# 0x002A/MuCHSALSA

Hardware: AMD Instinct MI355X
Metric: overlap-pairs/s (higher is better)
Workload: dtype int32+f64; 1 GPU; 100k synthetic Nanopore x10 kb, 500k unitig anchors, 10x coverage (BASELINE.json configs[2]); rows=5059558, reads=100000, anchors=499992, edges=981460, edgematches_rank0=25532466, orders_rank0=1029308, parallelism=one job on one GPU, edges_proven_clean_rank0=5372

## Files before the change

include/msgpu.h:

```cpp
#ifndef MSGPU_H
#define MSGPU_H

#include <stddef.h>
#include <stdint.h>

#ifdef __cplusplus
extern "C" {
#endif

#define MSGPU_VERSION 1

#define MSGPU_OK 0
#define MSGPU_E_IO (-1)
#define MSGPU_E_FORMAT (-2)
#define MSGPU_E_NUMBER (-3)
#define MSGPU_E_NOMEM (-4)
#define MSGPU_E_ARG (-5)
#define MSGPU_E_HIP (-6)
#define MSGPU_E_STATE (-7)
#define MSGPU_E_IDS (-8)
#define MSGPU_E_NODEVICE (-9)
#define MSGPU_E_LAYOUT (-10)
#define MSGPU_E_TIMEOUT (-11)

// ... 149 lines not shown
int msgpu_load_rows(msgpu_ctx *ctx, const msgpu_row *rows, size_t n_rows);
int msgpu_load_rows_packed(msgpu_ctx *ctx, const msgpu_packed_rows *packed);
int msgpu_load_rows_device(msgpu_ctx *ctx, const void *d_rows, size_t n_rows);


int msgpu_calculate_edges(msgpu_ctx *ctx);


int msgpu_chaining_and_overlaps(msgpu_ctx *ctx);


int msgpu_get_counts(msgpu_ctx *ctx, msgpu_counts *out);
int msgpu_get_timings(msgpu_ctx *ctx, msgpu_timings *out);
int msgpu_get_chain_band_counts(msgpu_ctx *ctx, uint64_t *n_banded, uint64_t *n_fallback);
int msgpu_chain_band_width(void);
int msgpu_set_stage_events(msgpu_ctx *ctx, int on);

int msgpu_copy_tables(msgpu_ctx *ctx, msgpu_edge *edges, msgpu_edgematch *ems, msgpu_order *orders, uint32_t *ids);
int msgpu_copy_tables_device(msgpu_ctx *ctx, void *d_edges, void *d_ems, void *d_orders, void *d_ids);
int msgpu_copy_reads(msgpu_ctx *ctx, int32_t *read_len, uint32_t *read_first_line);

int msgpu_merge_gathered(msgpu_ctx *ctx, const void *d_gathered, uint32_t world, const uint64_t *counts,
                         uint64_t slab_bytes, uint64_t off_edges, uint64_t off_orders, uint64_t off_ids, void *d_edges,
                         void *d_orders, void *d_ids);

int msgpu_merge_gathered_ex(msgpu_ctx *ctx, const void *d_gathered, uint32_t world, const uint64_t *counts,
                            uint64_t slab_bytes, uint64_t off_edges, uint64_t off_orders, uint64_t off_ids,
                            const uint32_t *id_base, void *d_edges, void *d_orders, void *d_ids, void *hip_stream);

uint64_t msgpu_wire_edges_bytes(uint64_t n_edges);
// ... 709 lines not shown
```

muchsalsa_amd/_lib.py:

```python
import ctypes as C
import os

import numpy as np

_HERE = os.path.dirname(os.path.abspath(__file__))
LIB_PATH = os.environ.get("MSGPU_LIB") or os.path.join(_HERE, "libmsgpu.so")

ROW_DTYPE = np.dtype([("anchor_id", "<u4"), ("read_id", "<u4"), ("read_len", "<i4"), ("i_lo", "<i4"),
                      ("i_hi", "<i4"), ("n_lo", "<i4"), ("n_hi", "<i4"), ("score", "<u4"), ("line", "<u4"),
                      ("flags", "<u4")])
EDGE_DTYPE = np.dtype([("v1", "<u4"), ("v2", "<u4"), ("em_off", "<u8"), ("order_off", "<u8"), ("em_cnt", "<u4"),
                       ("order_cnt", "<u2"), ("shadow", "u1"), ("pad", "u1")])
EM_DTYPE = np.dtype([("ov_lo", "<i4"), ("ov_hi", "<i4"), ("score", "<f8"), ("anchor_id", "<u4"), ("line", "<u4"),
                     ("flags", "<u4"), ("edge_idx", "<u4")])
ORDER_DTYPE = np.dtype([("edge_idx", "<u4"), ("flags", "<u4"), ("left_offset", "<f8"), ("right_offset", "<f8"),
                        ("score", "<u8"), ("ids_off", "<u8"), ("ids_cnt", "<u4"), ("start", "<u4"), ("end", "<u4"),
                        ("base", "<u4"), ("pad", "<u4", (2,))])
COPY_DTYPE = np.dtype([("src_off", "<u8"), ("dst_off", "<u8"), ("len", "<u4"), ("flags", "<u4")])
assert (ROW_DTYPE.itemsize, EDGE_DTYPE.itemsize, EM_DTYPE.itemsize, ORDER_DTYPE.itemsize) == (40, 32, 32, 64)
assert COPY_DTYPE.itemsize == 24
COPY_ILLUMINA, COPY_REVCOMP = 1, 2
PATH_READ_DTYPE = np.dtype([("read_id", "<u4"), ("direction", "<u4"), ("nanopore_length", "<u8")])
PATH_ORDER_DTYPE = np.dtype([("score", "<u8"), ("base_read", "<u4"), ("ids_off", "<u4"), ("ids_cnt", "<u4"),
                             ("pad", "<u4")])
# ... 297 lines not shown
    ("msgpu_paf_rows", C.c_void_p, [C.c_void_p, C.POINTER(C.c_size_t)]),
    ("msgpu_paf_line_count", C.c_size_t, [C.c_void_p]),
    ("msgpu_paf_read_count", C.c_uint32, [C.c_void_p]),
    ("msgpu_paf_anchor_count", C.c_uint32, [C.c_void_p]),
    ("msgpu_paf_read_name", C.c_char_p, [C.c_void_p, C.c_uint32]),
    ("msgpu_paf_anchor_name", C.c_char_p, [C.c_void_p, C.c_uint32]),
    ("msgpu_paf_register_sequences", C.c_int, [C.c_void_p, C.c_int, C.c_void_p, C.c_void_p, C.POINTER(C.c_uint32)]),
    ("msgpu_load_rows", C.c_int, [C.c_void_p, C.c_void_p, C.c_size_t]),
    ("msgpu_load_rows_device", C.c_int, [C.c_void_p, C.c_void_p, C.c_size_t]),
    ("msgpu_calculate_edges", C.c_int, [C.c_void_p]),
    ("msgpu_chaining_and_overlaps", C.c_int, [C.c_void_p]),
    ("msgpu_get_counts", C.c_int, [C.c_void_p, C.POINTER(Counts)]),
    ("msgpu_get_timings", C.c_int, [C.c_void_p, C.POINTER(Timings)]),
    ("msgpu_get_chain_band_counts", C.c_int, [C.c_void_p, C.POINTER(C.c_uint64), C.POINTER(C.c_uint64)]),
    ("msgpu_chain_band_width", C.c_int, []),
    ("msgpu_set_stage_events", C.c_int, [C.c_void_p, C.c_int]),
    ("msgpu_copy_tables", C.c_int, [C.c_void_p, C.c_void_p, C.c_void_p, C.c_void_p, C.c_void_p]),
    ("msgpu_copy_tables_device", C.c_int, [C.c_void_p, C.c_void_p, C.c_void_p, C.c_void_p, C.c_void_p]),
    ("msgpu_copy_reads", C.c_int, [C.c_void_p, C.c_void_p, C.c_void_p]),
    ("msgpu_merge_gathered", C.c_int, [C.c_void_p, C.c_void_p, C.c_uint32, C.c_void_p, C.c_uint64, C.c_uint64,
                                       C.c_uint64, C.c_uint64, C.c_void_p, C.c_void_p, C.c_void_p]),
    ("msgpu_merge_gathered_ex", C.c_int, [C.c_void_p, C.c_void_p, C.c_uint32, C.c_void_p, C.c_uint64, C.c_uint64,
                                          C.c_uint64, C.c_uint64, C.c_void_p, C.c_void_p, C.c_void_p, C.c_void_p,
                                          C.c_void_p]),
    ("msgpu_wire_edges_bytes", C.c_uint64, [C.c_uint64]),
    ("msgpu_wire_orders_bytes", C.c_uint64, [C.c_uint64]),
    ("msgpu_wire_ids_bytes", C.c_uint64, [C.c_uint64, C.c_uint32]),
    ("msgpu_pack_wire", C.c_int, [C.c_void_p, C.c_void_p, C.c_void_p, C.c_void_p, C.c_uint32]),
    ("msgpu_merge_wire", C.c_int, [C.c_void_p, C.c_void_p, C.c_uint32, C.c_void_p, C.c_uint64, C.c_uint64, C.c_uint64,
                                   C.c_uint64, C.c_uint32, C.c_void_p, C.c_void_p, C.c_void_p, C.c_void_p, C.c_void_p]),
# ... 274 lines not shown
```

muchsalsa_amd/csrc/msgpu_api.hip:

```cpp
#include <hip/hip_runtime.h>

#include <chrono>
#include <cmath>
#include <cstdarg>
#include <cstdio>
#include <cstdlib>
#include <cstring>
#include <condition_variable>
#include <deque>
#include <mutex>
#include <new>
#include <thread>
#include <vector>
#include <algorithm>
#include <sys/mman.h>
#include <unistd.h>

#include "asm_internal.h"
#include "host_pool.h"
#include "msgpu.h"
#include "msgpu_internal.h"
#include "msgpu_stage.h"

using namespace msgpu;
// ... 1162 lines not shown
int msgpu_get_chain_band_counts(msgpu_ctx *c, uint64_t *n_banded, uint64_t *n_fallback) {
  if (!c || !n_banded || !n_fallback) return MSGPU_E_ARG;
  *n_banded = *n_fallback = 0;
  if (c->state < ST_CHAINED || !c->chain_chunks.p) return MSGPU_OK;
  STAGE_HIP(c, hipSetDevice(c->device));
  const size_t n_chunks = static_cast<size_t>((c->chain_E + COMPACT_CHUNK - 1) / COMPACT_CHUNK);
  const size_t fb_word  = 2 * static_cast<size_t>(c->chain_E / COMPACT_CHUNK + 1);
  std::vector<unsigned long long> w(fb_word + 1);
  STAGE_HIP(c, hipStreamSynchronize(c->stream));
  STAGE_HIP(c, hipMemcpy(w.data(), c->chain_chunks.p, w.size() * 8, hipMemcpyDeviceToHost));
  for (size_t k = 0; k < n_chunks; ++k) *n_banded += (w[2 * k] >> 16) & 0xffffull;
  *n_fallback = w[fb_word];
  return MSGPU_OK;
}

int msgpu_get_timings(msgpu_ctx *c, msgpu_timings *out) {
  if (!c || !out) return MSGPU_E_ARG;
  memset(out, 0, sizeof(*out));
  STAGE_HIP(c, hipStreamSynchronize(c->stream));
  if (c->have_index_t) STAGE_HIP(c, hipEventElapsedTime(&out->index_ms, c->ev[0], c->ev[1]));
  if (c->have_cand_t) STAGE_HIP(c, hipEventElapsedTime(&out->candidates_ms, c->ev[2], c->ev[3]));
  if (c->have_chain_t) {
    if (c->have_stage_t) {
      STAGE_HIP(c, hipEventElapsedTime(&out->chain_ms, c->ev[4], c->ev[7]));
      STAGE_HIP(c, hipEventElapsedTime(&out->compact_ms, c->ev[7], c->ev[8]));
    }
    double   sum = 0;
    uint32_t n   = 0;
    for (uint32_t i = 0; i < c->ck_count; ++i) {
      const uint32_t slot = (c->ck_head + msgpu_ctx::CK_RING - 1 - i) % msgpu_ctx::CK_RING;
// ... 717 lines not shown
```

muchsalsa_amd/csrc/msgpu_device.h:

```cpp
#ifndef MSGPU_DEVICE_H
#define MSGPU_DEVICE_H

#include <hip/hip_runtime.h>
#include <stdint.h>

#include "msgpu.h"
#include "msgpu_internal.h"

namespace msgpu {

__device__ __forceinline__ IRow load_irow(const IRow *p) {
  const uint4 *q = reinterpret_cast<const uint4 *>(p);
  uint4        a = q[0], b = q[1];
  IRow         r;
  r.n_lo  = static_cast<int>(a.x);
  r.n_hi  = static_cast<int>(a.y);
  r.i_lo  = static_cast<int>(a.z);
  r.i_hi  = static_cast<int>(a.w);
  r.score = b.x;
  r.line  = b.y;
  r.other = b.z;
  r.pf    = b.w;
  return r;
}
// ... 155 lines not shown
    x = static_cast<long long>((static_cast<unsigned long long>(hi[0]) << 32) | lo[0]);
    y = static_cast<long long>((static_cast<unsigned long long>(hi[1]) << 32) | lo[1]);
    v = x > y ? x : y;
  }
  return v;
}
__device__ __forceinline__ double wave_prefix_max_f64(double v) {
  v = dpp_max_step<0x111>(v);
  v = dpp_max_step<0x112>(v);
  v = dpp_max_step<0x114>(v);
  v = dpp_max_step<0x118>(v);
  v = dpp_max_step<0x142, 0xa>(v);
  v = dpp_max_step<0x143, 0xc>(v);
  return v;
}

template <int NT> __device__ __forceinline__ uint32_t block_excl_scan(uint32_t v, uint32_t *s_wave , uint32_t *total) {
  const int      lane = threadIdx.x & 63, wave = threadIdx.x >> 6;
  const uint32_t inc  = wave_incl_scan(v);
  if (lane == 63) s_wave[wave] = inc;
  __syncthreads();
  uint32_t base = 0, tot = 0;
#pragma unroll
  for (int w = 0; w < NT / 64; ++w) {
    const uint32_t x = s_wave[w];
    base += w < wave ? x : 0u;
    tot += x;
  }
  *total = tot;
  __syncthreads();
// ... 110 lines not shown
```

muchsalsa_amd/csrc/msgpu_internal.h:

```cpp
#ifndef MSGPU_INTERNAL_H
#define MSGPU_INTERNAL_H

#include <hip/hip_runtime.h>
#include <stdint.h>

#include "msgpu.h"

namespace msgpu {

struct IRow {
  int32_t  n_lo, n_hi, i_lo, i_hi;
  uint32_t score, line, other, pf;
};
static_assert(sizeof(IRow) == 32, "IRow must be 32 bytes");
struct SRow {
  int32_t  i_lo, i_hi;
  uint32_t read, pf;
};
static_assert(sizeof(SRow) == 16, "SRow must be 16 bytes");
constexpr uint32_t PF_POS_MASK = 0x3fffffffu;
constexpr uint32_t PF_DIR      = 1u << 30;
constexpr uint32_t PF_PRIM     = 1u << 31;

enum { SC_MAXIDS = 0 , SC_ERR = 1, SC_TOTAL_A = 2, SC_TOTAL_B = 3, SC_TOTAL_C = 4, SC_NLISTS = 5 ,
// ... 220 lines not shown
void launch_classify_reads(hipStream_t st, const uint32_t *read_off, const uint32_t *read_cnt, const uint32_t *bound,
                           const uint64_t *cand_off, uint32_t V, uint32_t shard, uint32_t nshards, uint32_t lo,
                           uint32_t hi, CandDesc *l0, CandDesc *l1, CandDesc *l2, uint32_t *l3, uint32_t *n_lists, const CandZero &z,
                           unsigned long long *own_total = nullptr);
void launch_candidates(hipStream_t st, const CandArgs &a, int cls, const CandDesc *list, uint32_t n_list);
void launch_candidates_big(hipStream_t st, const CandArgs &a, const uint32_t *list, uint32_t n_list, uint64_t *big_key,
                           uint32_t *big_t, uint32_t *big_r2s, uint32_t *big_pfx);
void launch_emit_edges(hipStream_t st, const EmitArgs &a, bool reduce);
constexpr uint32_t PAIR_TAB_STRIDE = 2016 + 128;
#ifndef MSGPU_CHAIN_BAND
#define MSGPU_CHAIN_BAND 12
#endif
static_assert(MSGPU_CHAIN_BAND >= 1 && MSGPU_CHAIN_BAND <= 62, "band width");
constexpr int chain_band_pairs(int n) { return MSGPU_CHAIN_BAND * (MSGPU_CHAIN_BAND + 1) / 2 + (n - 1 - MSGPU_CHAIN_BAND) * MSGPU_CHAIN_BAND; }
static_assert(chain_band_pairs(64) <= 2016, "the band table fits the stride of the others");
constexpr uint32_t PAIR_TAB_BAND64_OFF = 4 * PAIR_TAB_STRIDE + 2 * PAIR_TAB_STRIDE + 3 * 2 * PAIR_TAB_STRIDE;
constexpr uint32_t PAIR_TAB_WORDS      = PAIR_TAB_BAND64_OFF + 2 * PAIR_TAB_STRIDE;
constexpr int CHAIN_FAST_SHORTCUT = 1, CHAIN_FAST_BAND = 2;
void launch_fill_pair_tab(hipStream_t st, uint32_t *tab);
void launch_chain(hipStream_t st, const ChainArgs &a, const uint32_t *list, uint32_t n_list);
void launch_chain_sub(hipStream_t st, const ChainArgs &a, int width, const uint32_t *list, uint32_t n_list);
struct ChainSubLists {
  const uint32_t *list32, *list16, *list8;
  uint32_t        n32, n16, n8, nb32, nb16;
};
void launch_chain_sub_all(hipStream_t st, const ChainArgs &a, const uint32_t *l32, uint32_t n32, const uint32_t *l16, uint32_t n16,
                          const uint32_t *l8, uint32_t n8);
size_t big_elem_bytes();
size_t big_path_bytes();
void launch_chain_big(hipStream_t st, const ChainArgs &a, const uint32_t *big_list, const uint64_t *big_off,
                      uint32_t n_big, void *elems, void *paths);
void launch_merge_gathered(hipStream_t st, const MergeArgs &a);
// ... 35 lines not shown
```

muchsalsa_amd/csrc/msgpu_kernels.hip:

```cpp
#include <hip/hip_runtime.h>
#include <stdint.h>
#include <stdlib.h>

#include <type_traits>
#include <utility>

#include "msgpu.h"
#include "msgpu_internal.h"
#include "msgpu_device.h"

namespace msgpu {


constexpr int SCAN_ITEMS = 8;
uint32_t      scan_blocks(uint64_t n);

template <class T> __global__ __launch_bounds__(256) void k_scan_reduce(const uint32_t *in, uint64_t n, T *block_sums) {
  __shared__ T s[4];
  uint64_t     base = static_cast<uint64_t>(blockIdx.x) * 256 * SCAN_ITEMS;
  T            sum  = 0;
  for (int i = 0; i < SCAN_ITEMS; ++i) {
    uint64_t idx = base + static_cast<uint64_t>(i) * 256 + threadIdx.x;
    if (idx < n) sum += in[idx];
  }
// ... 1279 lines not shown
        a.big_off[i]  = atomicAdd(&a.big_cursor[1], static_cast<unsigned long long>(ed.em_cnt));
      } else if (ed.em_cnt) {
        a.list[atomicAdd(&s_pos[ed.em_cnt - 1], 1u)] = static_cast<uint32_t>(eb + e);
      }
    }
  }
}
void launch_emit_edges(hipStream_t st, const EmitArgs &a, bool reduce) {
  if (reduce && a.n_chunks)
    hipLaunchKernelGGL(k_cand_reduce, dim3(a.n_chunks), dim3(1024), 0, st, a.n_edge, a.n_cand, a.cand_off, a.edge_scr_start, a.V,
                       const_cast<unsigned long long *>(a.chunk_sums), const_cast<uint32_t *>(a.hist));
  hipLaunchKernelGGL(k_emit_edges, dim3(a.n_chunks ? a.n_chunks : 1), dim3(1024), 0, st, a);
}


__device__ __forceinline__ void chunk_add(unsigned long long *chunk_sums, uint64_t e, bool clean, uint32_t n_orders, uint32_t n_ids, bool banded = false) {
  static_assert(COMPACT_CHUNK < (1u << 16), "two 16-bit edge counts in the low half of a chunk sum");
  unsigned long long *c = chunk_sums + 2 * (e / COMPACT_CHUNK);
  __hip_atomic_fetch_add(c, (clean ? 1ull : 0ull) | (banded ? 1ull << 16 : 0ull) | (static_cast<unsigned long long>(n_orders) << 32), __ATOMIC_RELAXED, __HIP_MEMORY_SCOPE_AGENT);
  __hip_atomic_fetch_add(c + 1, static_cast<unsigned long long>(n_ids), __ATOMIC_RELAXED, __HIP_MEMORY_SCOPE_AGENT);
}
__device__ __forceinline__ void edge_counts(msgpu_edge *edges, uint64_t e, uint32_t em_cnt, uint32_t n_orders, uint32_t n_ids, bool shadow) {
  reinterpret_cast<uint4 *>(&edges[e])[1] = make_uint4(n_ids, 0u, em_cnt, (n_orders & 0xffffu) | (shadow ? 1u << 16 : 0u));
}
__device__ __forceinline__ void band_fallback_add(unsigned long long *chunk_sums, uint64_t n_edges) {
  __hip_atomic_fetch_add(chunk_sums + 2 * (n_edges / COMPACT_CHUNK + 1), 1ull, __ATOMIC_RELAXED, __HIP_MEMORY_SCOPE_AGENT);
}

struct PathRec {
  uint64_t mask;
  uint64_t score;
  uint32_t primary;
  uint32_t pad;
};

struct __attribute__((aligned(16))) ChainElem {
  double clo1, chi1;
  double clo2, chi2;
  int    rlo1, rhi1, rlo2, rhi2;
};

// ... 646 lines not shown
  const int      wave = threadIdx.x >> 6, lane = threadIdx.x & 63;
  const int      g = lane / W, sl = lane % W, gbase = g * W;
  const uint32_t slot    = (block * 4 + wave) * G + g;
  const bool     valid_g = slot < n_list;
  if (__ballot(valid_g) == 0) return;
  const uint32_t   e  = valid_g ? list[slot] : list[0];
  const msgpu_edge ed = a.edges[e];
  const uint32_t   n  = (valid_g && ed.em_cnt <= static_cast<uint32_t>(W)) ? ed.em_cnt : 0u;
  const uint64_t   cp = a.edge_cand[e];
  const bool       act = sl < static_cast<int>(n);
  const uint32_t   v1 = ed.v1, v2 = ed.v2;
  const uint32_t   n1 = a.read_cnt[v1], n2 = a.read_cnt[v2];
  const int        len1 = a.read_len[v1], len2 = a.read_len[v2];
  ChainElem       *el = reinterpret_cast<ChainElem *>(s_wavebuf[wave]);
  uint32_t        *cm = s_cm[wave];

  uint32_t  j1 = 0, q2 = 0, anchor = 0;
  double    clo1 = 0, clo2 = 0, ovr1 = 0, ovr2 = 0, em_score = 0;
  bool      em_dir = false, em_prim = false;
  ChainElem x{};
  cm[lane] = 0;
  if (act) {
    j1            = a.cand_j[cp + sl];
    const uint32_t qt = a.cand_q[cp + sl];
    const IRow m1 = load_irow(&a.by_read[a.read_off[v1] + j1]);
    const IRow m2 = load_irow(&a.by_read[a.read_off[v2] + qt]);
    anchor        = m1.other;
    const int  ov_lo = max(m1.i_lo, m2.i_lo), ov_hi = min(m1.i_hi, m2.i_hi);
    const bool d1 = (m1.pf & PF_DIR) != 0, d2 = (m2.pf & PF_DIR) != 0;
    em_dir           = d1 == d2;
// ... 76 lines not shown
      int a_hi = act ? static_cast<int>(ceil(av)) : -2147483647 - 1;
      int a_lo = act ? static_cast<int>(floor(av)) : 2147483647;
      int b_hi = act ? static_cast<int>(ceil(bv)) : -2147483647 - 1;
      int b_lo = act ? static_cast<int>(floor(bv)) : 2147483647;
#pragma unroll
      for (int d = W / 2; d > 0; d >>= 1) {
        a_hi = max(a_hi, __shfl_xor(a_hi, d));
        a_lo = min(a_lo, __shfl_xor(a_lo, d));
        b_hi = max(b_hi, __shfl_xor(b_hi, d));
        b_lo = min(b_lo, __shfl_xor(b_lo, d));
      }
      clean = maybe && static_cast<long long>(a_hi) - b_lo <= a.fast_margin && static_cast<long long>(b_hi) - a_lo <= a.fast_margin;
    }
  }

  const int P = clean ? 0 : static_cast<int>(n * (n - 1) / 2);
  const int nP   = longest_prefix<W>(__ballot(act && !clean));
  const int Pmax = nP * (nP - 1) / 2;
  const bool               one_dir = __ballot(m_plus != 0 && m_minus != 0) == 0;
  const unsigned long long KD_one  = __ballot(m_minus == 0);
  static_assert(sizeof(ChainElem) == 48, "the pair table holds byte offsets of 48-byte elements");
  const __amdgpu_buffer_rsrc_t tab_rsrc = __builtin_amdgcn_make_buffer_rsrc(
      const_cast<uint32_t *>(a.pair_tab_sub) + (W == 32 ? 0 : W == 16 ? 1 : 2) * PAIR_TAB_STRIDE * 2, 0, PAIR_TAB_STRIDE * 8, 0x00020000);
  const uint32_t tab_lane = static_cast<uint32_t>(sl) * 8u;
  auto           load_pairs = [&](int p0) __attribute__((always_inline)) -> uint2 {
    typedef int v2i __attribute__((ext_vector_type(2)));
    const v2i   v = __builtin_amdgcn_raw_buffer_load_b64(tab_rsrc, tab_lane, p0 * 8, 0);
    return make_uint2(static_cast<uint32_t>(v.x), static_cast<uint32_t>(v.y));
  };
  const int            Pl  = P - sl;
  const unsigned char *elg = reinterpret_cast<const unsigned char *>(el + gbase);
  unsigned char       *cmg = reinterpret_cast<unsigned char *>(cm + gbase);
  double          wiggle  = a.wiggle;
  asm volatile("" : "+v"(wiggle));
  bool wf_lane = true;
  if (act) {
    const int prev_rlo1 = el[sl > 0 ? lane - 1 : lane].rlo1;
    wf_lane = (x.clo1 <= x.chi1) & (x.clo2 <= x.chi2) & (x.rlo1 <= x.rhi1) & (sl == 0 || prev_rlo1 <= x.rlo1);
  }
  const bool wf = __ballot(!wf_lane) == 0;
  auto sweep_step = [&](int p0, const uint2 kl, auto wft, auto dirt) __attribute__((always_inline)) {
    typedef decltype(wft)  WFT;
    typedef decltype(dirt) DIRT;
    constexpr int          DIR = DIRT::value;
    unsigned long long     bits;
    const bool             in_range = p0 < Pl;
    {
      typedef unsigned long long M;
      M valid = __ballot(in_range), KD = KD_one;
      if (DIR == 2) {
        const int  k = static_cast<int>(kl.y & 0xffu), l = static_cast<int>(kl.y >> 18);
        const bool kd = (m_plus >> k) & 1u, ld = (m_plus >> l) & 1u;
        valid &= __ballot(kd == ld);
        KD    = __ballot(kd);
      }
// ... 47 lines not shown
    }
  };
  auto sweep_dir = [&](auto wft) __attribute__((always_inline)) {
    if (!one_dir) sweep(wft, std::integral_constant<int, 2>{});
    else if (KD_one == ~0ull) sweep(wft, std::integral_constant<int, 0>{});
    else if (KD_one == 0) sweep(wft, std::integral_constant<int, 1>{});
    else sweep(wft, std::integral_constant<int, 3>{});
  };
  if (wf) sweep_dir(std::true_type{});
  else sweep_dir(std::false_type{});
  __builtin_amdgcn_fence(__ATOMIC_RELEASE, "wavefront");
  __builtin_amdgcn_wave_barrier();
  const uint32_t mycm = clean ? (act ? (1u << sl) - 1u : 0u) : cm[lane];

  const int nmax = longest_prefix<W>(__ballot(act));
  double    pop  = em_score;
  uint32_t  pm   = 1u << sl;
  {
    uint32_t pred = static_cast<uint32_t>(sl);
    uint32_t rev  = __builtin_bitreverse32(mycm);
    auto     dp_step = [&](double cand, int k) __attribute__((always_inline)) {
      unsigned long long comp, saved;
      asm volatile("v_add_co_u32 %0, %1, %0, %0" : "+v"(rev), "=s"(comp));
      const unsigned long long upd = comp & __ballot(cand > pop);
      asm volatile("s_and_saveexec_b64 %[sv], %[m]\n\t"
                   "v_mov_b64 %[pop], %[cand]\n\t"
                   "v_mov_b32 %[pred], %[k]\n\t"
                   "s_mov_b64 exec, %[sv]"
                   : [pop] "+v"(pop), [pred] "+v"(pred), [sv] "=&s"(saved)
                   : [m] "s"(upd), [cand] "v"(cand), [k] "s"(k)
                   : "scc");
    };
// ... 7 lines not shown
        std::make_integer_sequence<int, W - 1>{});
    uint32_t ptr = pred;
    for (int span = 1; span < nmax; span <<= 1) {
      if constexpr (W == 32) {
        const uint32_t o  = __shfl(pm, gbase + static_cast<int>(ptr));
        const uint32_t p2 = __shfl(ptr, gbase + static_cast<int>(ptr));
        pm |= o;
        ptr = p2;
      } else {
        const uint32_t o = __shfl(pm | (ptr << 16), gbase + static_cast<int>(ptr));
        pm |= o & 0xffffu;
        ptr = o >> 16;
      }
    }
  }

  SubPath *pmn = reinterpret_cast<SubPath *>(s_wavebuf[wave]) + gbase, *ppl = pmn + 64;
  uint32_t n_m = 0, n_p = 0;
#pragma clang loop unroll(disable)
  for (int trip = 0; trip < 2; ++trip) {
    const bool     dir  = trip != 0 || m_minus == 0;
    const uint32_t actd = trip == 0 ? (m_minus ? m_minus : m_plus) : (m_minus ? m_plus : 0u);
    const uint32_t np   = paths_of_direction_sub<W>(actd, dir, sl, gbase, pop, pm, em_prim, j1, q2, n1, n2, a.alt_frac, dir ? ppl : pmn);
    if (actd) (dir ? n_p : n_m) = np;
    if (__ballot(m_minus != 0 && m_plus != 0) == 0) break;
  }
  __builtin_amdgcn_fence(__ATOMIC_RELEASE, "wavefront");
  __builtin_amdgcn_wave_barrier();

  bool     k_m = false, k_p = false;
  uint32_t prim_m = 0, prim_p = 0, len_m = 0, len_p = 0;
  if (sl < static_cast<int>(n_m)) {
    prim_m = pmn[sl].primary;
    len_m  = static_cast<uint32_t>(__popc(pmn[sl].mask));
    k_m    = true;
  }
  if (sl < static_cast<int>(n_p)) {
    prim_p = ppl[sl].primary;
// ... 46 lines not shown
        ro   = R1 - R2;
      } else if (L1 > L2 && R1 < R2) {
        have = true;
        fl   = MSGPU_ORD_START_V1;
        lo   = L1 - L2;
        ro   = R2 - R1;
      } else if (L1 < L2 && R1 > R2) {
        have = true;
        fl   = 0;
        lo   = L2 - L1;
        ro   = R1 - R2;
      }
      const bool emit = has && have;
      if (emit) {
        const uint32_t cnt = static_cast<uint32_t>(__popc(mask));
        if ((mask >> sl) & 1u) a.ids_scr[ed.em_off + n_ids + static_cast<uint32_t>(__popc(mask & ((1u << sl) - 1u)))] = s_anchor[wave][lane];
        if (sl == 0) {
          msgpu_order o;
          o.edge_idx     = e;
          o.flags        = fl | (dir ? MSGPU_ORD_DIR : 0u) | (rec.primary ? MSGPU_ORD_PRIMARY : 0u);
          o.left_offset  = lo;
          o.right_offset = ro;
          o.score        = rec.score;
          o.ids_off      = n_ids;
          o.ids_cnt      = cnt;
          o.start        = (fl & MSGPU_ORD_START_V1) ? v1 : v2;
          o.end          = (fl & MSGPU_ORD_START_V1) ? v2 : v1;
          o.base         = v1;
          o.pad[0]       = 0;
          o.pad[1]       = 0;
          a.order_scr[ed.em_off + n_orders] = o;
        }
        ++n_orders;
        n_ids += cnt;
      }
    }
  }
  if (n && sl == 0) {
    edge_counts(a.edges, e, n, n_orders, n_ids, shadow);
    chunk_add(a.chunk_sums, e, clean, n_orders, n_ids);
  }
}

template <int W>
__global__ __launch_bounds__(256) __attribute__((amdgpu_waves_per_eu(W == 32 ? 7 : 6, W == 32 ? 7 : 6))) void k_chain_sub(ChainArgs a, const uint32_t *list, uint32_t n_list) {
  __shared__ __attribute__((aligned(16))) unsigned char s_wavebuf[4][sizeof(ChainElem) * 64];
  __shared__ uint32_t                                  s_cm[4][64];
  __shared__ __attribute__((aligned(16))) double       s_keep[4][64][4];
  __shared__ uint32_t                                  s_anchor[4][64];
  chain_sub_body<W>(a, list, n_list, blockIdx.x, s_wavebuf, s_cm, s_keep, s_anchor);
}
#ifndef MSGPU_SUB_WAVES
#define MSGPU_SUB_WAVES 7
#endif
__global__ __launch_bounds__(256) __attribute__((amdgpu_waves_per_eu(MSGPU_SUB_WAVES, MSGPU_SUB_WAVES))) void k_chain_sub_all(ChainArgs a, ChainSubLists l) {
// ... 471 lines not shown
    if (l * (l - 1) / 2 > p) --l;
    if ((l + 1) * l / 2 <= p) ++l;
    k = p - l * (l - 1) / 2;
  } else {
    const int q = p - TRI;
    l = B + 1 + q / B;
    k = l - B + q % B;
    if (l >= 64) {
      k = 0;
      l = 1;
    }
  }
  tab[PAIR_TAB_BAND64_OFF + 2 * p]     = static_cast<uint32_t>(k * 48);
  tab[PAIR_TAB_BAND64_OFF + 2 * p + 1] = static_cast<uint32_t>(l * 48);
}
__global__ __launch_bounds__(256) void k_fill_pair_tab(uint32_t *tab) {
  const int i = blockIdx.x * 256 + threadIdx.x;
  if (i >= 4 * static_cast<int>(PAIR_TAB_STRIDE)) return;
  const int t = i / static_cast<int>(PAIR_TAB_STRIDE), p = i % static_cast<int>(PAIR_TAB_STRIDE), W = 64 >> t;
  if (t == 0) band64_entry(tab, p);
  if (p >= 2016) {
    tab[i] = 1u << 8;
    if (t == 0) tab64_entry(tab, p, 0, 1, 0);
    else tabsub_entry(tab, t, p, 0, 1, 0);
    return;
  }
  int l = static_cast<int>((1.0f + __fsqrt_rn(1.0f + 8.0f * static_cast<float>(p))) * 0.5f);
  if (l * (l - 1) / 2 > p) --l;
  if ((l + 1) * l / 2 <= p) ++l;
  const int k = p - l * (l - 1) / 2, lane = p % W;
  const int run = (k == 0 || lane == 0) ? min(l - k, W - lane) : 0;
  tab[i] = static_cast<uint32_t>(k | (l << 8) | (run << 16)) | (static_cast<uint32_t>(64 - run - k) << 24);
  if (t == 0) tab64_entry(tab, p, k, l, run);
  else tabsub_entry(tab, t, p, k, l, run);
}
// ... 12 lines not shown
  static_assert(COMPACT_CHUNK == 1024, "an edge per thread");
  const int      lane = threadIdx.x & 63, wave = threadIdx.x >> 6;
  const uint32_t chunk = blockIdx.x;
  const uint64_t my_e = static_cast<uint64_t>(chunk) * COMPACT_CHUNK + threadIdx.x;
  uint4          my_lo = make_uint4(0, 0, 0, 0), my_hi = make_uint4(0, 0, 0, 0);
  if (my_e < a.n_edges) {
    const uint4 *p = reinterpret_cast<const uint4 *>(&a.edges[my_e]);
    my_lo          = p[0];
    my_hi          = p[1];
  }
  static_assert(sizeof(msgpu_edge) == 32 && offsetof(msgpu_edge, em_off) == 8 && offsetof(msgpu_edge, order_off) == 16 &&
                    offsetof(msgpu_edge, em_cnt) == 24 && offsetof(msgpu_edge, order_cnt) == 28,
                "the edge record as two 16-byte halves");
  unsigned long long t[5] = {0, 0, 0, 0, 0};
  for (uint32_t c = threadIdx.x; c < a.n_chunks; c += 1024) {
    const unsigned long long w0 = a.chunk_sums[2 * c], w1 = a.chunk_sums[2 * c + 1];
    const unsigned long long no = w0 >> 32, nf = w0 & 0xffffull;
    if (c < chunk) {
      t[0] += no;
      t[1] += w1;
    }
    t[2] += no;
    t[3] += w1;
    t[4] += nf;
  }
#pragma unroll
  for (int k = 0; k < 5; ++k) {
    for (int d = 32; d > 0; d >>= 1) t[k] += __shfl_xor(t[k], d);
    if (lane == 0) s_red[wave][k] = t[k];
  }
  __syncthreads();
// ... 457 lines not shown
```

muchsalsa_amd/overlap.py:

```python
import ctypes as C
import os

import numpy as np

from . import _lib
from ._lib import EDGE_DTYPE, EM_DTYPE, ORDER_DTYPE, ROW_DTYPE, Counts, HostTables, Params, Timings


class MsgpuError(RuntimeError):
    def __init__(self, code, detail=""):
        msg = _lib.lib().msgpu_strerror(code).decode()
        super().__init__("%s (%d)%s" % (msg, code, (": " + detail) if detail else ""))
        self.code = code


def default_params():
    p = Params()
    _lib.lib().msgpu_default_params(C.byref(p))
    return p


class Paf:

    def __init__(self, rows, n_lines, read_names, anchor_names, handle=None, n_reads=None, n_anchors=None):
# ... 174 lines not shown
        self._check(self._L.msgpu_synchronize(self._h))

    def counts(self):
        c = Counts()
        self._check(self._L.msgpu_get_counts(self._h, C.byref(c)))
        return c

    def chain_band_counts(self):
        nb, nf = C.c_uint64(0), C.c_uint64(0)
        self._check(self._L.msgpu_get_chain_band_counts(self._h, C.byref(nb), C.byref(nf)))
        return int(nb.value), int(nf.value)

    def chain_band_width(self):
        return int(self._L.msgpu_chain_band_width())

    def set_stage_events(self, on):
        self._check(self._L.msgpu_set_stage_events(self._h, 1 if on else 0))

    def timings(self):
        t = Timings()
        self._check(self._L.msgpu_get_timings(self._h, C.byref(t)))
        return t

    def tables(self):
        c = self.counts()
        edges = np.zeros(c.n_edges, dtype=EDGE_DTYPE)
        ems = np.zeros(c.n_ems, dtype=EM_DTYPE)
        orders = np.zeros(c.n_orders, dtype=ORDER_DTYPE)
        ids = np.zeros(c.n_ids, dtype="<u4")
        self._check(self._L.msgpu_copy_tables(self._h, edges.ctypes.data, ems.ctypes.data, orders.ctypes.data,
# ... 173 lines not shown
```

Baseline: 472.5 million overlap-pairs/s.

## Add banded chaining with verify-and-redo fallback for 32-wide sub-wavefront edges

For edges handled by the 32-lane sub-wavefront chain kernel with at least MSGPU_SUB_BAND_MIN elements, the DP now only considers predecessor pairs within a band of MSGPU_SUB_BAND, using a new banded pair table. A prefix-max check confirms that no out-of-band predecessor could beat the banded result, and any half-wave that fails the check reruns the full all-pairs sweep. The aim is to cut the quadratic pair work on long chains. The cost is an extra verification pass, a possible redo loop, and edge fields staged in shared memory to keep register pressure down. Counters for banded and redone edges are packed into the high bits of the chunk sums and exposed through new API calls.

```diff
diff --git a/include/msgpu.h b/include/msgpu.h
--- a/include/msgpu.h
+++ b/include/msgpu.h
@@ -187,6 +187,9 @@
 int msgpu_get_timings(msgpu_ctx *ctx, msgpu_timings *out);
 int msgpu_get_chain_band_counts(msgpu_ctx *ctx, uint64_t *n_banded, uint64_t *n_fallback);
 int msgpu_chain_band_width(void);
+int msgpu_get_chain_sub_band_counts(msgpu_ctx *ctx, uint64_t *n_banded, uint64_t *n_redone);
+int msgpu_chain_sub_band_width(void);
+int msgpu_chain_sub_band_min(void);
 int msgpu_set_stage_events(msgpu_ctx *ctx, int on);
 
 int msgpu_copy_tables(msgpu_ctx *ctx, msgpu_edge *edges, msgpu_edgematch *ems, msgpu_order *orders, uint32_t *ids);
diff --git a/muchsalsa_amd/_lib.py b/muchsalsa_amd/_lib.py
--- a/muchsalsa_amd/_lib.py
+++ b/muchsalsa_amd/_lib.py
@@ -335,6 +335,9 @@
     ("msgpu_get_timings", C.c_int, [C.c_void_p, C.POINTER(Timings)]),
     ("msgpu_get_chain_band_counts", C.c_int, [C.c_void_p, C.POINTER(C.c_uint64), C.POINTER(C.c_uint64)]),
     ("msgpu_chain_band_width", C.c_int, []),
+    ("msgpu_get_chain_sub_band_counts", C.c_int, [C.c_void_p, C.POINTER(C.c_uint64), C.POINTER(C.c_uint64)]),
+    ("msgpu_chain_sub_band_width", C.c_int, []),
+    ("msgpu_chain_sub_band_min", C.c_int, []),
     ("msgpu_set_stage_events", C.c_int, [C.c_void_p, C.c_int]),
     ("msgpu_copy_tables", C.c_int, [C.c_void_p, C.c_void_p, C.c_void_p, C.c_void_p, C.c_void_p]),
     ("msgpu_copy_tables_device", C.c_int, [C.c_void_p, C.c_void_p, C.c_void_p, C.c_void_p, C.c_void_p]),
diff --git a/muchsalsa_amd/csrc/msgpu_api.hip b/muchsalsa_amd/csrc/msgpu_api.hip
--- a/muchsalsa_amd/csrc/msgpu_api.hip
+++ b/muchsalsa_amd/csrc/msgpu_api.hip
@@ -1200,6 +1200,24 @@
   return MSGPU_OK;
 }
 
+int msgpu_chain_sub_band_width(void) { return MSGPU_SUB_BAND; }
+int msgpu_chain_sub_band_min(void) { return MSGPU_SUB_BAND_MIN; }
+
+int msgpu_get_chain_sub_band_counts(msgpu_ctx *c, uint64_t *n_banded, uint64_t *n_redone) {
+  if (!c || !n_banded || !n_redone) return MSGPU_E_ARG;
+  *n_banded = *n_redone = 0;
+  if (c->state < ST_CHAINED || !c->chain_chunks.p) return MSGPU_OK;
+  STAGE_HIP(c, hipSetDevice(c->device));
+  const size_t n_chunks = static_cast<size_t>((c->chain_E + COMPACT_CHUNK - 1) / COMPACT_CHUNK);
+  const size_t fb_word  = 2 * static_cast<size_t>(c->chain_E / COMPACT_CHUNK + 1);
+  std::vector<unsigned long long> w(fb_word + 2);
+  STAGE_HIP(c, hipStreamSynchronize(c->stream));
+  STAGE_HIP(c, hipMemcpy(w.data(), c->chain_chunks.p, w.size() * 8, hipMemcpyDeviceToHost));
+  for (size_t k = 0; k < n_chunks; ++k) *n_banded += w[2 * k + 1] >> 48;
+  *n_redone = w[fb_word + 1];
+  return MSGPU_OK;
+}
+
 int msgpu_get_timings(msgpu_ctx *c, msgpu_timings *out) {
   if (!c || !out) return MSGPU_E_ARG;
   memset(out, 0, sizeof(*out));
diff --git a/muchsalsa_amd/csrc/msgpu_device.h b/muchsalsa_amd/csrc/msgpu_device.h
--- a/muchsalsa_amd/csrc/msgpu_device.h
+++ b/muchsalsa_amd/csrc/msgpu_device.h
@@ -193,6 +193,14 @@
   v = dpp_max_step<0x143, 0xc>(v);
   return v;
 }
+__device__ __forceinline__ double half_prefix_max_f64(double v) {
+  v = dpp_max_step<0x111>(v);
+  v = dpp_max_step<0x112>(v);
+  v = dpp_max_step<0x114>(v);
+  v = dpp_max_step<0x118>(v);
+  v = dpp_max_step<0x142, 0xa>(v);
+  return v;
+}
 
 template <int NT> __device__ __forceinline__ uint32_t block_excl_scan(uint32_t v, uint32_t *s_wave , uint32_t *total) {
   const int      lane = threadIdx.x & 63, wave = threadIdx.x >> 6;
diff --git a/muchsalsa_amd/csrc/msgpu_internal.h b/muchsalsa_amd/csrc/msgpu_internal.h
--- a/muchsalsa_amd/csrc/msgpu_internal.h
+++ b/muchsalsa_amd/csrc/msgpu_internal.h
@@ -258,8 +258,18 @@
 static_assert(MSGPU_CHAIN_BAND >= 1 && MSGPU_CHAIN_BAND <= 62, "band width");
 constexpr int chain_band_pairs(int n) { return MSGPU_CHAIN_BAND * (MSGPU_CHAIN_BAND + 1) / 2 + (n - 1 - MSGPU_CHAIN_BAND) * MSGPU_CHAIN_BAND; }
 static_assert(chain_band_pairs(64) <= 2016, "the band table fits the stride of the others");
-constexpr uint32_t PAIR_TAB_BAND64_OFF = 4 * PAIR_TAB_STRIDE + 2 * PAIR_TAB_STRIDE + 3 * 2 * PAIR_TAB_STRIDE;
-constexpr uint32_t PAIR_TAB_WORDS      = PAIR_TAB_BAND64_OFF + 2 * PAIR_TAB_STRIDE;
+#ifndef MSGPU_SUB_BAND
+#define MSGPU_SUB_BAND 10
+#endif
+#ifndef MSGPU_SUB_BAND_MIN
+#define MSGPU_SUB_BAND_MIN 20
+#endif
+static_assert(MSGPU_SUB_BAND >= 1 && MSGPU_SUB_BAND_MIN >= MSGPU_SUB_BAND + 2 && MSGPU_SUB_BAND_MIN <= 33, "sub-wavefront band");
+constexpr int chain_sub_band_pairs(int n) { return MSGPU_SUB_BAND * (MSGPU_SUB_BAND + 1) / 2 + (n - 1 - MSGPU_SUB_BAND) * MSGPU_SUB_BAND; }
+constexpr uint32_t PAIR_TAB_SUB_OFF    = 4 * PAIR_TAB_STRIDE + 2 * PAIR_TAB_STRIDE;
+constexpr uint32_t PAIR_TAB_BAND64_OFF = PAIR_TAB_SUB_OFF + 3 * 2 * PAIR_TAB_STRIDE;
+constexpr uint32_t PAIR_TAB_BAND32_OFF = PAIR_TAB_BAND64_OFF + 2 * PAIR_TAB_STRIDE;
+constexpr uint32_t PAIR_TAB_WORDS      = PAIR_TAB_BAND32_OFF + 2 * PAIR_TAB_STRIDE;
 constexpr int CHAIN_FAST_SHORTCUT = 1, CHAIN_FAST_BAND = 2;
 void launch_fill_pair_tab(hipStream_t st, uint32_t *tab);
 void launch_chain(hipStream_t st, const ChainArgs &a, const uint32_t *list, uint32_t n_list);
diff --git a/muchsalsa_amd/csrc/msgpu_kernels.hip b/muchsalsa_amd/csrc/msgpu_kernels.hip
--- a/muchsalsa_amd/csrc/msgpu_kernels.hip
+++ b/muchsalsa_amd/csrc/msgpu_kernels.hip
@@ -1317,17 +1317,19 @@
 }
 
 
-__device__ __forceinline__ void chunk_add(unsigned long long *chunk_sums, uint64_t e, bool clean, uint32_t n_orders, uint32_t n_ids, bool banded = false) {
+constexpr unsigned long long CHUNK_IDS_MASK = (1ull << 48) - 1;
+__device__ __forceinline__ void chunk_add(unsigned long long *chunk_sums, uint64_t e, bool clean, uint32_t n_orders, uint32_t n_ids, bool banded = false,
+                                          bool sub_banded = false) {
   static_assert(COMPACT_CHUNK < (1u << 16), "two 16-bit edge counts in the low half of a chunk sum");
   unsigned long long *c = chunk_sums + 2 * (e / COMPACT_CHUNK);
   __hip_atomic_fetch_add(c, (clean ? 1ull : 0ull) | (banded ? 1ull << 16 : 0ull) | (static_cast<unsigned long long>(n_orders) << 32), __ATOMIC_RELAXED, __HIP_MEMORY_SCOPE_AGENT);
-  __hip_atomic_fetch_add(c + 1, static_cast<unsigned long long>(n_ids), __ATOMIC_RELAXED, __HIP_MEMORY_SCOPE_AGENT);
+  __hip_atomic_fetch_add(c + 1, static_cast<unsigned long long>(n_ids) | (sub_banded ? 1ull << 48 : 0ull), __ATOMIC_RELAXED, __HIP_MEMORY_SCOPE_AGENT);
 }
 __device__ __forceinline__ void edge_counts(msgpu_edge *edges, uint64_t e, uint32_t em_cnt, uint32_t n_orders, uint32_t n_ids, bool shadow) {
   reinterpret_cast<uint4 *>(&edges[e])[1] = make_uint4(n_ids, 0u, em_cnt, (n_orders & 0xffffu) | (shadow ? 1u << 16 : 0u));
 }
-__device__ __forceinline__ void band_fallback_add(unsigned long long *chunk_sums, uint64_t n_edges) {
-  __hip_atomic_fetch_add(chunk_sums + 2 * (n_edges / COMPACT_CHUNK + 1), 1ull, __ATOMIC_RELAXED, __HIP_MEMORY_SCOPE_AGENT);
+__device__ __forceinline__ void band_fallback_add(unsigned long long *chunk_sums, uint64_t n_edges, bool sub = false) {
+  __hip_atomic_fetch_add(chunk_sums + 2 * (n_edges / COMPACT_CHUNK + 1) + (sub ? 1 : 0), 1ull, __ATOMIC_RELAXED, __HIP_MEMORY_SCOPE_AGENT);
 }
 
 struct PathRec {
@@ -2004,6 +2006,13 @@
   const int        len1 = a.read_len[v1], len2 = a.read_len[v2];
   ChainElem       *el = reinterpret_cast<ChainElem *>(s_wavebuf[wave]);
   uint32_t        *cm = s_cm[wave];
+  __shared__ __attribute__((aligned(16))) uint32_t s_edge[4][2][8];
+  if constexpr (W == 32) {
+    if (sl == 0) {
+      *reinterpret_cast<uint4 *>(s_edge[wave][g])     = make_uint4(v1, v2, static_cast<uint32_t>(ed.em_off), static_cast<uint32_t>(ed.em_off >> 32));
+      *reinterpret_cast<uint2 *>(s_edge[wave][g] + 4) = make_uint2(n1, n2);
+    }
+  }
 
   uint32_t  j1 = 0, q2 = 0, anchor = 0;
   double    clo1 = 0, clo2 = 0, ovr1 = 0, ovr2 = 0, em_score = 0;
@@ -2110,16 +2119,42 @@
     }
   }
 
-  const int P = clean ? 0 : static_cast<int>(n * (n - 1) / 2);
-  const int nP   = longest_prefix<W>(__ballot(act && !clean));
-  const int Pmax = nP * (nP - 1) / 2;
+  constexpr bool     BANDW    = W == 32;
+  constexpr uint32_t BAND_TAB = (PAIR_TAB_BAND32_OFF - PAIR_TAB_SUB_OFF) * 4u;
+  unsigned long long band_m = 0, redo_m = 0;
+  if constexpr (BANDW) band_m = __ballot(!clean && (a.fast_path & CHAIN_FAST_BAND) && n >= static_cast<uint32_t>(MSGPU_SUB_BAND_MIN));
+  const unsigned long long banded_m = band_m;
   const bool               one_dir = __ballot(m_plus != 0 && m_minus != 0) == 0;
   const unsigned long long KD_one  = __ballot(m_minus == 0);
   static_assert(sizeof(ChainElem) == 48, "the pair table holds byte offsets of 48-byte elements");
+  static_assert(PAIR_TAB_BAND32_OFF > PAIR_TAB_SUB_OFF, "the 32-wide band table lies behind the full one");
   const __amdgpu_buffer_rsrc_t tab_rsrc = __builtin_amdgcn_make_buffer_rsrc(
-      const_cast<uint32_t *>(a.pair_tab_sub) + (W == 32 ? 0 : W == 16 ? 1 : 2) * PAIR_TAB_STRIDE * 2, 0, PAIR_TAB_STRIDE * 8, 0x00020000);
-  const uint32_t tab_lane = static_cast<uint32_t>(sl) * 8u;
-  auto           load_pairs = [&](int p0) __attribute__((always_inline)) -> uint2 {
+      const_cast<uint32_t *>(a.pair_tab_sub) + (W == 32 ? 0 : W == 16 ? 1 : 2) * PAIR_TAB_STRIDE * 2, 0,
+      BANDW ? (PAIR_TAB_BAND32_OFF - PAIR_TAB_SUB_OFF) * 4 + PAIR_TAB_STRIDE * 8 : PAIR_TAB_STRIDE * 8, 0x00020000);
+  bool wf_lane = true;
+  if (act) {
+    const int prev_rlo1 = el[sl > 0 ? lane - 1 : lane].rlo1;
+    wf_lane = (x.clo1 <= x.chi1) & (x.clo2 <= x.chi2) & (x.rlo1 <= x.rhi1) & (sl == 0 || prev_rlo1 <= x.rlo1);
+  }
+  const bool wf = __ballot(!wf_lane) == 0;
+  double     pop;
+  uint32_t   pm;
+  for (;;) {
+  int      P        = clean ? 0 : static_cast<int>(n * (n - 1) / 2);
+  uint32_t tab_lane = static_cast<uint32_t>(sl) * 8u;
+  int      Pmax;
+  if constexpr (BANDW) {
+    if ((band_m >> lane) & 1ull) {
+      P = chain_sub_band_pairs(static_cast<int>(n));
+      tab_lane += BAND_TAB;
+    }
+    if (redo_m != 0 && !((redo_m >> lane) & 1ull)) P = 0;
+    Pmax = max(__builtin_amdgcn_readlane(P, 0), __builtin_amdgcn_readlane(P, 32));
+  } else {
+    const int nP = longest_prefix<W>(__ballot(act && !clean));
+    Pmax         = nP * (nP - 1) / 2;
+  }
+  auto          load_pairs = [&](int p0) __attribute__((always_inline)) -> uint2 {
     typedef int v2i __attribute__((ext_vector_type(2)));
     const v2i   v = __builtin_amdgcn_raw_buffer_load_b64(tab_rsrc, tab_lane, p0 * 8, 0);
     return make_uint2(static_cast<uint32_t>(v.x), static_cast<uint32_t>(v.y));
@@ -2129,12 +2164,6 @@
   unsigned char       *cmg = reinterpret_cast<unsigned char *>(cm + gbase);
   double          wiggle  = a.wiggle;
   asm volatile("" : "+v"(wiggle));
-  bool wf_lane = true;
-  if (act) {
-    const int prev_rlo1 = el[sl > 0 ? lane - 1 : lane].rlo1;
-    wf_lane = (x.clo1 <= x.chi1) & (x.clo2 <= x.chi2) & (x.rlo1 <= x.rhi1) & (sl == 0 || prev_rlo1 <= x.rlo1);
-  }
-  const bool wf = __ballot(!wf_lane) == 0;
   auto sweep_step = [&](int p0, const uint2 kl, auto wft, auto dirt) __attribute__((always_inline)) {
     typedef decltype(wft)  WFT;
     typedef decltype(dirt) DIRT;
@@ -2212,8 +2241,8 @@
   const uint32_t mycm = clean ? (act ? (1u << sl) - 1u : 0u) : cm[lane];
 
   const int nmax = longest_prefix<W>(__ballot(act));
-  double    pop  = em_score;
-  uint32_t  pm   = 1u << sl;
+  pop = em_score;
+  pm  = 1u << sl;
   {
     uint32_t pred = static_cast<uint32_t>(sl);
     uint32_t rev  = __builtin_bitreverse32(mycm);
@@ -2251,14 +2280,40 @@
       }
     }
   }
-
+  if constexpr (!BANDW) {
+    break;
+  } else {
+    if (band_m == 0) break;
+    const double pmax = half_prefix_max_f64(pop);
+    const double out  = shfl_f64(pmax, gbase + (sl > MSGPU_SUB_BAND ? sl - MSGPU_SUB_BAND - 1 : 0));
+    const unsigned long long rej_m = __ballot(sl > MSGPU_SUB_BAND && act && !(out + em_score < pop)) & band_m;
+    if (rej_m == 0) break;
+    redo_m = (static_cast<uint32_t>(rej_m) ? 0xffffffffull : 0ull) | ((rej_m >> 32) ? 0xffffffff00000000ull : 0ull);
+    band_m = 0;
+    if (((redo_m >> lane) & 1ull) && sl == 0) band_fallback_add(a.chunk_sums, a.n_edges, true);
+    __builtin_amdgcn_fence(__ATOMIC_RELEASE, "wavefront");
+    __builtin_amdgcn_wave_barrier();
+  }
+  }
+
+  uint32_t e_again = e;
+  asm volatile("" : "+v"(e_again));
+  uint4 pk0 = make_uint4(0, 0, 0, 0);
+  uint2 pk1 = make_uint2(0, 0);
+  if constexpr (BANDW) {
+    pk0 = *reinterpret_cast<const uint4 *>(s_edge[wave][g]);
+    pk1 = *reinterpret_cast<const uint2 *>(s_edge[wave][g] + 4);
+  }
+  const uint32_t v1_ = BANDW ? pk0.x : v1, v2_ = BANDW ? pk0.y : v2;
+  const uint64_t em_off_ = BANDW ? static_cast<uint64_t>(pk0.z) | (static_cast<uint64_t>(pk0.w) << 32) : ed.em_off;
+  const uint32_t n1_ = BANDW ? pk1.x : n1, n2_ = BANDW ? pk1.y : n2;
   SubPath *pmn = reinterpret_cast<SubPath *>(s_wavebuf[wave]) + gbase, *ppl = pmn + 64;
   uint32_t n_m = 0, n_p = 0;
 #pragma clang loop unroll(disable)
   for (int trip = 0; trip < 2; ++trip) {
     const bool     dir  = trip != 0 || m_minus == 0;
     const uint32_t actd = trip == 0 ? (m_minus ? m_minus : m_plus) : (m_minus ? m_plus : 0u);
-    const uint32_t np   = paths_of_direction_sub<W>(actd, dir, sl, gbase, pop, pm, em_prim, j1, q2, n1, n2, a.alt_frac, dir ? ppl : pmn);
+    const uint32_t np   = paths_of_direction_sub<W>(actd, dir, sl, gbase, pop, pm, em_prim, j1, q2, n1_, n2_, a.alt_frac, dir ? ppl : pmn);
     if (actd) (dir ? n_p : n_m) = np;
     if (__ballot(m_minus != 0 && m_plus != 0) == 0) break;
   }
@@ -2335,7 +2390,7 @@
       const bool emit = has && have;
       if (emit) {
         const uint32_t cnt = static_cast<uint32_t>(__popc(mask));
-        if ((mask >> sl) & 1u) a.ids_scr[ed.em_off + n_ids + static_cast<uint32_t>(__popc(mask & ((1u << sl) - 1u)))] = s_anchor[wave][lane];
+        if ((mask >> sl) & 1u) a.ids_scr[em_off_ + n_ids + static_cast<uint32_t>(__popc(mask & ((1u << sl) - 1u)))] = s_anchor[wave][lane];
         if (sl == 0) {
           msgpu_order o;
           o.edge_idx     = e;
@@ -2345,12 +2400,12 @@
           o.score        = rec.score;
           o.ids_off      = n_ids;
           o.ids_cnt      = cnt;
-          o.start        = (fl & MSGPU_ORD_START_V1) ? v1 : v2;
-          o.end          = (fl & MSGPU_ORD_START_V1) ? v2 : v1;
-          o.base         = v1;
+          o.start        = (fl & MSGPU_ORD_START_V1) ? v1_ : v2_;
+          o.end          = (fl & MSGPU_ORD_START_V1) ? v2_ : v1_;
+          o.base         = v1_;
           o.pad[0]       = 0;
           o.pad[1]       = 0;
-          a.order_scr[ed.em_off + n_orders] = o;
+          a.order_scr[em_off_ + n_orders] = o;
         }
         ++n_orders;
         n_ids += cnt;
@@ -2358,8 +2413,8 @@
     }
   }
   if (n && sl == 0) {
-    edge_counts(a.edges, e, n, n_orders, n_ids, shadow);
-    chunk_add(a.chunk_sums, e, clean, n_orders, n_ids);
+    edge_counts(a.edges, BANDW ? e_again : e, n, n_orders, n_ids, shadow);
+    chunk_add(a.chunk_sums, e, clean, n_orders, n_ids, false, BANDW && ((banded_m >> lane) & 1ull));
   }
 }
 
@@ -2861,11 +2916,33 @@
   tab[PAIR_TAB_BAND64_OFF + 2 * p]     = static_cast<uint32_t>(k * 48);
   tab[PAIR_TAB_BAND64_OFF + 2 * p + 1] = static_cast<uint32_t>(l * 48);
 }
+__device__ __forceinline__ void band32_entry(uint32_t *tab, int p) {
+  constexpr int B = MSGPU_SUB_BAND, TRI = B * (B + 1) / 2;
+  int k = 0, l = 1, k0 = 0;
+  if (p < TRI) {
+    l = static_cast<int>((1.0f + __fsqrt_rn(1.0f + 8.0f * static_cast<float>(p))) * 0.5f);
+    if (l * (l - 1) / 2 > p) --l;
+    if ((l + 1) * l / 2 <= p) ++l;
+    k = p - l * (l - 1) / 2;
+  } else {
+    const int q = p - TRI;
+    l  = B + 1 + q / B;
+    k0 = l - B;
+    k  = k0 + q % B;
+  }
+  const int lane = p % 32;
+  int       run  = (k == k0 || lane == 0) ? min(l - k, 32 - lane) : 0;
+  if (l >= 32) k = 0, l = 1, run = 0;
+  uint32_t *e = tab + PAIR_TAB_BAND32_OFF + 2 * p;
+  e[0]        = static_cast<uint32_t>(k * 48) | (static_cast<uint32_t>(l * 48) << 16);
+  e[1]        = static_cast<uint32_t>(k) | (static_cast<uint32_t>(run) << 8) | (static_cast<uint32_t>(l * 4) << 16);
+}
 __global__ __launch_bounds__(256) void k_fill_pair_tab(uint32_t *tab) {
   const int i = blockIdx.x * 256 + threadIdx.x;
   if (i >= 4 * static_cast<int>(PAIR_TAB_STRIDE)) return;
   const int t = i / static_cast<int>(PAIR_TAB_STRIDE), p = i % static_cast<int>(PAIR_TAB_STRIDE), W = 64 >> t;
   if (t == 0) band64_entry(tab, p);
+  if (t == 1) band32_entry(tab, p);
   if (p >= 2016) {
     tab[i] = 1u << 8;
     if (t == 0) tab64_entry(tab, p, 0, 1, 0);
@@ -2908,7 +2985,7 @@
                 "the edge record as two 16-byte halves");
   unsigned long long t[5] = {0, 0, 0, 0, 0};
   for (uint32_t c = threadIdx.x; c < a.n_chunks; c += 1024) {
-    const unsigned long long w0 = a.chunk_sums[2 * c], w1 = a.chunk_sums[2 * c + 1];
+    const unsigned long long w0 = a.chunk_sums[2 * c], w1 = a.chunk_sums[2 * c + 1] & CHUNK_IDS_MASK;
     const unsigned long long no = w0 >> 32, nf = w0 & 0xffffull;
     if (c < chunk) {
       t[0] += no;
diff --git a/muchsalsa_amd/overlap.py b/muchsalsa_amd/overlap.py
--- a/muchsalsa_amd/overlap.py
+++ b/muchsalsa_amd/overlap.py
@@ -212,6 +212,14 @@
     def chain_band_width(self):
         return int(self._L.msgpu_chain_band_width())
 
+    def chain_sub_band_counts(self):
+        nb, nr = C.c_uint64(0), C.c_uint64(0)
+        self._check(self._L.msgpu_get_chain_sub_band_counts(self._h, C.byref(nb), C.byref(nr)))
+        return int(nb.value), int(nr.value)
+
+    def chain_sub_band(self):
+        return int(self._L.msgpu_chain_sub_band_width()), int(self._L.msgpu_chain_sub_band_min())
+
     def set_stage_events(self, on):
         self._check(self._L.msgpu_set_stage_events(self._h, 1 if on else 0))
 
```

Result: no change. 479.6 million overlap-pairs/s (median of 6 runs) (+1.5%).
